# carrenD/Medical-Cross-Modality-Domain-Adaptation

Measured on AMD Instinct MI355X. Metric: training slices/sec (256x256x3, B=16/GPU) joint segmenter+GAN step (1 dis update on B MR + B CT, clip, 1 gen update on B CT), higher is better.
Workload: dtype f32; 1 GPU; BASELINE configs[3]: train_gan.py --phase train-gan joint step, B=16/GPU per domain, f32, dropout .75, mask critic on; global_batch=16, per_gpu_batch=16, parallelism=dp1, step_capture=False

## Files before the change

include/pnp_hip.h:

```cpp
#ifndef PNP_HIP_H
#define PNP_HIP_H

#include <stddef.h>
#include <stdint.h>

#ifdef __cplusplus
extern "C" {
#endif

#define PNP_OK 0
#define PNP_EINVAL (-1)
#define PNP_ELAUNCH (-2)
#define PNP_EWORKSPACE (-3)
#define PNP_ECOMM (-4)

#define PNP_DTYPE_F32 0
#define PNP_DTYPE_BF16 1
#define PNP_DTYPE_F64 2

#define PNP_PAD_ZERO 0
#define PNP_PAD_SYMMETRIC 1

int pnp_abi_version(void);
const char* pnp_last_error(void);
// ... 30 lines not shown

int32_t pnp_conv2d_fwd_stats_parts(const pnp_conv_geom* g);
int pnp_conv2d_fwd_stats(const float* x, const float* w, float* y, const pnp_conv_geom* g,
                         float keep_prob, uint64_t seed, uint32_t stream_id,
                         const float* shift , float* parts, size_t parts_bytes, void* stream);
int32_t pnp_conv2d_fwd_stats_ws_parts(const pnp_conv_geom* g);
int pnp_conv2d_fwd_stats_ws(const float* x, const float* w, float* y, const pnp_conv_geom* g,
                            float keep_prob, uint64_t seed, uint32_t stream_id,
                            const float* shift , float* parts, size_t parts_bytes,
                            void* workspace, size_t workspace_bytes, void* stream);
int32_t pnp_conv2d_wino_chosen(const pnp_conv_geom* g, int32_t kind);
int32_t pnp_conv2d_wino_mode(int32_t mode);
int32_t pnp_conv2d_wino_tile(int32_t tile);
int32_t pnp_conv2d_wino_x3(int32_t mode);
int32_t pnp_conv2d_x3_direct(int32_t mode);
size_t pnp_conv2d_wino_filter_bytes(int32_t C, int32_t K);
int pnp_conv2d_wino_filter_bind(const float* w, int32_t kind, float* U, size_t bytes);
void pnp_weights_changed(const void* lo, const void* hi);
void pnp_conv2d_wino_filter_stats(int64_t* hits, int64_t* fills, int32_t reset);
int32_t pnp_conv2d_wino_wgrad_mode(int32_t mode);

int pnp_bn_fold(const float* gamma, const float* beta, const float* mean, const float* var, float* scale, float* shift,
                int32_t C, float eps, void* stream);
int pnp_conv2d_fwd_bn(const float* x, const float* w, float* y, const pnp_conv_geom* g,
                      float keep_prob, uint64_t seed, uint32_t stream_id,
                      const float* scale, const float* shift, const float* shortcut , int32_t Cs, float alpha,
                      void* stream);
int pnp_conv2d_fwd_bn_ws(const float* x, const float* w, float* y, const pnp_conv_geom* g,
                         float keep_prob, uint64_t seed, uint32_t stream_id,
                         const float* scale, const float* shift, const float* shortcut , int32_t Cs, float alpha,
// ... 160 lines not shown
```

medical-cross-modality-domain-adaptation_amd/_lib.py:

```python
import ctypes
import os

import torch

from ctypes import POINTER, c_char_p, c_float, c_int, c_int32, c_int64, c_size_t, c_uint32, c_uint64, c_void_p

_HERE = os.path.dirname(os.path.abspath(__file__))
LIB_PATH = os.environ.get("PNP_LIB") or os.path.join(_HERE, "libpnp_hip.so")

PAD_ZERO = 0
PAD_SYMMETRIC = 1
OPT_CHUNK = 1024
DTYPE_F32, DTYPE_BF16, DTYPE_F64 = 0, 1, 2
COMM_ID_BYTES = 128
ABI_VERSION = 4


class ConvGeom(ctypes.Structure):
    _fields_ = [(n, c_int32) for n in
                ("N", "H", "W", "C", "K", "R", "S", "OH", "OW", "stride", "dil", "pad_t", "pad_l", "pad_mode", "dtype")]

    def key(self):
        return tuple(getattr(self, f) for f, _ in self._fields_)

# ... 30 lines not shown
    "pnp_conv2d_fwd_ws": (c_int, [_F, _F, _F, _G, c_float, c_uint64, c_uint32, c_void_p, c_size_t, c_void_p]),
    "pnp_conv2d_fwd_stats_parts": (c_int32, [_G]),
    "pnp_conv2d_fwd_stats": (c_int, [_F, _F, _F, _G, c_float, c_uint64, c_uint32, _F, _F, c_size_t, c_void_p]),
    "pnp_bn_stats_finish": (c_int, [_F, c_int32, _F, _F, _F, _F, _F, c_int64, c_int32, c_float, c_void_p]),
    "pnp_bn_fold": (c_int, [_F, _F, _F, _F, _F, _F, c_int32, c_float, c_void_p]),
    "pnp_conv2d_fwd_bn": (c_int, [_F, _F, _F, _G, c_float, c_uint64, c_uint32, _F, _F, _F, c_int32, c_float, c_void_p]),
    "pnp_conv2d_fwd_bn_ws": (c_int, [_F, _F, _F, _G, c_float, c_uint64, c_uint32, _F, _F, _F, c_int32, c_float, c_void_p, c_size_t, c_void_p]),
    "pnp_conv2d_fwd_stats_ws_parts": (c_int32, [_G]),
    "pnp_conv2d_fwd_stats_ws": (c_int, [_F, _F, _F, _G, c_float, c_uint64, c_uint32, _F, _F, c_size_t, c_void_p, c_size_t, c_void_p]),
    "pnp_conv2d_wino_chosen": (c_int32, [_G, c_int32]),
    "pnp_conv2d_wino_mode": (c_int32, [c_int32]),
    "pnp_conv2d_wino_wgrad_mode": (c_int32, [c_int32]),
    "pnp_conv2d_wino_tile": (c_int32, [c_int32]),
    "pnp_conv2d_wino_x3": (c_int32, [c_int32]),
    "pnp_conv2d_x3_direct": (c_int32, [c_int32]),
    "pnp_conv2d_wino_filter_bytes": (c_size_t, [c_int32, c_int32]),
    "pnp_conv2d_wino_filter_bind": (c_int, [c_void_p, c_int32, c_void_p, c_size_t]),
    "pnp_weights_changed": (None, [c_void_p, c_void_p]),
    "pnp_conv2d_wino_filter_stats": (None, [POINTER(c_int64), POINTER(c_int64), c_int32]),
    "pnp_conv2d_fwd_naive": (c_int, [_F, _F, _F, _G, c_void_p]),
    "pnp_dropout": (c_int, [_F, _F, c_size_t, c_float, c_uint64, c_uint32, c_void_p]),
    "pnp_bn_workspace_bytes": (c_size_t, [c_int64, c_int32]),
    "pnp_bn_stats": (c_int, [_F, _F, _F, c_int64, c_int32, c_void_p, c_size_t, c_void_p]),
    "pnp_bn_stats_update": (c_int, [_F, _F, _F, _F, _F, c_int64, c_int32, c_float, c_void_p, c_size_t, c_void_p]),
    "pnp_bn_update_moving": (c_int, [_F, _F, _F, _F, c_int64, c_int32, c_float, c_void_p]),
    "pnp_bn_apply": (c_int, [_F, _F, _F, _F, _F, _F, c_int32, _F, c_int64, c_int32, c_float, c_float, c_void_p]),
    "pnp_bn_bwd": (c_int, [_F, _F, _F, _F, _F, _F, _F, _F, _F, _F, _F, c_int32, c_int64, c_int32, c_float, c_float, c_int32,
                           c_float, c_uint64, c_uint32, c_void_p, c_size_t, c_void_p]),
    "pnp_bn_bwd_acc": (c_int, [_F, _F, _F, _F, _F, _F, _F, _F, _F, _F, _F, _F, _F, c_int32, c_int64, c_int32, c_float, c_float, c_int32,
                               c_float, c_uint64, c_uint32, c_void_p, c_size_t, c_void_p]),
# ... 112 lines not shown
```

medical-cross-modality-domain-adaptation_amd/csrc/conv_common.h:

```cpp
#pragma once
#include "pnp_common.h"

namespace pnpconv {

constexpr int BK = 32;
constexpr int NTHREADS = 256;
#ifndef PNP_CONV_ABLATE
#define PNP_CONV_ABLATE 0
#endif
constexpr int kAblate = PNP_CONV_ABLATE;

struct ConvArgs {
    const float* x;
    const float* w;
    float* y;
    int N, H, W, C, K, R, S, OH, OW, stride, dil, pad_t, pad_l, pad_mode;
    int ups;
    int M;
    int Kred;
    int OHW;
    int nblk_m, nblk_n;
    int gn;
    int nsplit, chunks_per_split;
    long long split_stride;
// ... 288 lines not shown
    size_t wt_off;
};
int plan_phases(const pnp_conv_geom* g, DgradPhase* ph);
pnp_conv_geom phase_geom(const pnp_conv_geom* g, const DgradPhase& p);
bool n16_geom_ok(const pnp_conv_geom* g);
bool n16_wgrad_ok(const pnp_conv_geom* g);
int launch_n16_fwd(const ConvArgs& a, int kind, hipStream_t st);
int n16_wgrad_blocks(const pnp_conv_geom* g);
int launch_n16_wgrad(const ConvArgs& a, float* part, hipStream_t st);
bool wino_eligible(const pnp_conv_geom* g);
bool x3d_chosen(const pnp_conv_geom* g);
bool x3d_chosen(const ConvArgs& a);
int x3d_stats_parts(const pnp_conv_geom* g);
size_t x3d_filter_bytes(int C, int K);
int launch_x3_direct(const ConvArgs& a, int kind, bool flip_transpose, void* ws, size_t ws_bytes, hipStream_t st);
bool wino_chosen(const pnp_conv_geom* g);
int wino_tile(const pnp_conv_geom* g);
size_t wino_workspace_bytes(const pnp_conv_geom* g);
int wino_stats_parts(const pnp_conv_geom* g);
int launch_wino(const ConvArgs& a, int kind, bool flip_transpose, void* ws, size_t ws_bytes, hipStream_t st);
bool wino_wgrad_chosen(const pnp_conv_geom* g);
int wino_wgrad_tile(const pnp_conv_geom* g);
size_t wino_wgrad_workspace_bytes(const pnp_conv_geom* g);
int launch_wino_wgrad(const ConvArgs& a, float* dw, int accumulate, void* ws, size_t ws_bytes, hipStream_t st);
#ifndef PNP_X3_SW
#define PNP_X3_SW 32
#endif
constexpr int X3_SW = PNP_X3_SW;
static_assert(X3_SW == 16 || X3_SW == 32, "stage width");
bool wino_x3_dims_ok(int T, int C, int K);
// ... 10 lines not shown
```

medical-cross-modality-domain-adaptation_amd/csrc/conv_igemm.hip:

```cpp
#include "conv_common.h"
#include "conv_mma.h"

using namespace pnpconv;

#ifdef PNP_TRACE
constexpr int TRACE_WG = 512, TRACE_N = 192;
__device__ unsigned long long g_trace[TRACE_WG][TRACE_N];
#define PNP_TRACE_MARK(slot)                                                                             \
    do {                                                                                                 \
        const unsigned tr_ = blockIdx.x - (gridDim.x > 4352u ? 4096u : 0u);        \
        if (threadIdx.x == 0 && tr_ < (unsigned)TRACE_WG && (slot) < TRACE_N) g_trace[tr_][(slot)] = __builtin_readcyclecounter(); \
    } while (0)
extern "C" int pnp_debug_trace_read(void* host, size_t bytes) {
    if (bytes > sizeof(unsigned long long) * TRACE_WG * TRACE_N) bytes = sizeof(unsigned long long) * TRACE_WG * TRACE_N;
    return hipMemcpyFromSymbol(host, HIP_SYMBOL(g_trace), bytes, 0, hipMemcpyDeviceToHost) == hipSuccess ? 0 : -1;
}
#else
#define PNP_TRACE_MARK(slot) do { } while (0)
#endif

namespace {

template <int BN, bool VEC>
struct BLoader {
// ... 1895 lines not shown
        flops += 2.0 * rows * g->C * (double)(p.T * p.U * g->K);
        bytes += 4.0 * (rows * g->C + (double)p.T * p.U * g->K * g->C);
    }
    ga.nph = n;
    if (n == 0) return PNP_OK;
    bytes += 4.0 * (double)g->N * g->OH * g->OW * g->K;
    PnpProfScope ps(PNP_PROF_CONV_DGRAD, st, flops, bytes, "conv_dgrad_phases_kernel<128, %d, %d, %d>", bn, narrow ? 4 : 2, narrow ? 1 : 2);
    if (narrow) hipLaunchKernelGGL((conv_dgrad_phases_kernel<128, 32, 4, 1>), dim3((unsigned)blk), dim3(NTHREADS), 0, st, ga);
    else hipLaunchKernelGGL((conv_dgrad_phases_kernel<128, 64, 2, 2>), dim3((unsigned)blk), dim3(NTHREADS), 0, st, ga);
    PNP_CHECK_LAUNCH("conv_dgrad_phases_kernel");
    return PNP_OK;
}

}

extern "C" {

static int fwd_split(const pnp_conv_geom* g) {
    if (g->pad_mode != PNP_PAD_ZERO) return 1;
    const long long M = (long long)g->N * g->OH * g->OW;
    const int tile = choose_tile(M, g->K);
    const int bn = tile == 0 ? 128 : (tile == 1 ? 64 : 32);
    if ((long long)pnp_cdiv(M, 128) * pnp_cdiv(g->K, bn) > 128) return 1;
    return choose_split(M, g->K, g->R * g->S * g->C, tile);
}

size_t pnp_conv2d_fwd_workspace_bytes(const pnp_conv_geom* g) {
    if (!g) return 0;
    if (wino_chosen(g)) return wino_workspace_bytes(g);
    const int ns = fwd_split(g);
    const size_t split = ns > 1 ? (size_t)ns * g->N * g->OH * g->OW * g->K * sizeof(float) : 0;
    const size_t x3d = x3d_chosen(g) ? x3d_filter_bytes(g->C, g->K) : 0;
    return split > x3d ? split : x3d;
}

int pnp_conv2d_fwd(const float* x, const float* w, float* y, const pnp_conv_geom* g, float keep_prob, uint64_t seed,
                   uint32_t stream_id, void* stream) {
    return pnp_conv2d_fwd_ws(x, w, y, g, keep_prob, seed, stream_id, nullptr, 0, stream);
}

int pnp_conv2d_fwd_ws(const float* x, const float* w, float* y, const pnp_conv_geom* g, float keep_prob, uint64_t seed,
                      uint32_t stream_id, void* workspace, size_t workspace_bytes, void* stream) {
    if (int e = check_geom(g, "pnp_conv2d_fwd")) return e;
    PNP_REQUIRE(x && w && y, "pnp_conv2d_fwd: null pointer");
    PNP_REQUIRE(keep_prob > 0.f, "pnp_conv2d_fwd: keep_prob must be > 0");
    ConvArgs a = make_args(x, w, y, g);
    if (keep_prob < 1.f) {
        a.do_drop = 1;
        a.drop_keep = keep_prob;
        a.drop_key = pnp_drop_key(seed, stream_id);
        a.drop_thresh = pnp_drop_thresh(keep_prob);
        a.sp = pnp_step_params_ptr(); a.drop_sid = stream_id;
    }
    if (n16_geom_ok(g)) return launch_n16_fwd(a, 0, (hipStream_t)stream);
    if (narrow_fwd_ok(g, nullptr)) return launch_narrow(x, w, y, g, a, (hipStream_t)stream);
    if (wino_chosen(g)) {
        if (workspace && workspace_bytes >= wino_workspace_bytes(g)) return launch_wino(a, 0, false, workspace, workspace_bytes, (hipStream_t)stream);
        return launch_fwd<0>(a, (hipStream_t)stream, nullptr);
    }
    if (x3d_chosen(a) && workspace && workspace_bytes >= x3d_filter_bytes(a.C, a.K))
        return launch_x3_direct(a, 0, false, workspace, workspace_bytes, (hipStream_t)stream);
    float* split_ws = (workspace && workspace_bytes >= pnp_conv2d_fwd_workspace_bytes(g) && pnp_conv2d_fwd_workspace_bytes(g) > 0)
                          ? (float*)workspace : nullptr;
    return launch_fwd<0>(a, (hipStream_t)stream, split_ws);
}

static int fwd_stats_impl(const float* x, const float* w, float* y, const pnp_conv_geom* g, float keep_prob, uint64_t seed,
                          uint32_t stream_id, const float* shift, float* parts, size_t parts_bytes, void* workspace, size_t workspace_bytes,
                          void* stream, bool with_ws);

int32_t pnp_conv2d_fwd_stats_parts(const pnp_conv_geom* g) {
    if (!g || check_geom(g, "pnp_conv2d_fwd_stats_parts") != PNP_OK) return 0;
    if (n16_geom_ok(g) || narrow_fwd_ok(g, nullptr) || fwd_split(g) > 1) return 0;
    const long long M = (long long)g->N * g->OH * g->OW;
    const int tile = choose_tile(M, g->K);
    return pnp_cdiv(M, 128) * ((tile == 0 || tile == 1) ? 2 : 4);
}

int pnp_conv2d_fwd_stats(const float* x, const float* w, float* y, const pnp_conv_geom* g, float keep_prob, uint64_t seed,
                         uint32_t stream_id, const float* shift, float* parts, size_t parts_bytes, void* stream) {
    return fwd_stats_impl(x, w, y, g, keep_prob, seed, stream_id, shift, parts, parts_bytes, nullptr, 0, stream, false);
}

int32_t pnp_conv2d_fwd_stats_ws_parts(const pnp_conv_geom* g) {
    if (!g || check_geom(g, "pnp_conv2d_fwd_stats_ws_parts") != PNP_OK) return 0;
    if (wino_chosen(g)) return wino_stats_parts(g);
    if (x3d_chosen(g) && !n16_geom_ok(g) && !narrow_fwd_ok(g, nullptr)) return x3d_stats_parts(g);
    return pnp_conv2d_fwd_stats_parts(g);
}

int pnp_conv2d_fwd_stats_ws(const float* x, const float* w, float* y, const pnp_conv_geom* g, float keep_prob, uint64_t seed,
                            uint32_t stream_id, const float* shift, float* parts, size_t parts_bytes, void* workspace,
                            size_t workspace_bytes, void* stream) {
    return fwd_stats_impl(x, w, y, g, keep_prob, seed, stream_id, shift, parts, parts_bytes, workspace, workspace_bytes, stream, true);
}

static int fwd_stats_impl(const float* x, const float* w, float* y, const pnp_conv_geom* g, float keep_prob, uint64_t seed,
                          uint32_t stream_id, const float* shift, float* parts, size_t parts_bytes, void* workspace, size_t workspace_bytes,
                          void* stream, bool with_ws) {
    if (int e = check_geom(g, "pnp_conv2d_fwd_stats")) return e;
    PNP_REQUIRE(x && w && y && parts, "pnp_conv2d_fwd_stats: null pointer");
    PNP_REQUIRE(keep_prob > 0.f, "pnp_conv2d_fwd_stats: keep_prob must be > 0");
    const bool wino = with_ws && wino_chosen(g);
    if (wino) PNP_REQUIRE(workspace && workspace_bytes >= wino_workspace_bytes(g), "pnp_conv2d_fwd_stats_ws: workspace too small (pnp_conv2d_fwd_workspace_bytes)");
    const bool x3d = with_ws && !wino && x3d_chosen(g) && !n16_geom_ok(g) && !narrow_fwd_ok(g, nullptr);
    if (x3d) PNP_REQUIRE(workspace && workspace_bytes >= x3d_filter_bytes(g->C, g->K), "pnp_conv2d_fwd_stats_ws: workspace too small (pnp_conv2d_fwd_workspace_bytes)");
    const int nparts = wino ? wino_stats_parts(g) : (x3d ? x3d_stats_parts(g) : pnp_conv2d_fwd_stats_parts(g));
    PNP_REQUIRE(nparts > 0, "pnp_conv2d_fwd_stats: no epilogue statistics for this geometry (pnp_conv2d_fwd_stats_parts == 0)");
    if (parts_bytes < (size_t)nparts * 2 * g->K * sizeof(float)) {
        pnp_set_error("pnp_conv2d_fwd_stats: parts buffer too small (%zu < %zu)", parts_bytes, (size_t)nparts * 2 * g->K * sizeof(float));
        return PNP_EWORKSPACE;
    }
    ConvArgs a = make_args(x, w, y, g);
    if (keep_prob < 1.f) {
        a.do_drop = 1;
        a.drop_keep = keep_prob;
        a.drop_key = pnp_drop_key(seed, stream_id);
        a.drop_thresh = pnp_drop_thresh(keep_prob);
        a.sp = pnp_step_params_ptr(); a.drop_sid = stream_id;
    }
    a.stat_ws = parts;
    a.stat_shift = shift;
    if (wino) return launch_wino(a, 0, false, workspace, workspace_bytes, (hipStream_t)stream);
    if (x3d) return launch_x3_direct(a, 0, false, workspace, workspace_bytes, (hipStream_t)stream);
    return launch_fwd<0>(a, (hipStream_t)stream);
}

int pnp_bn_fold(const float* gamma, const float* beta, const float* mean, const float* var, float* scale, float* shift, int32_t C,
                float eps, void* stream) {
    PNP_REQUIRE(gamma && beta && mean && var && scale && shift && C > 0, "pnp_bn_fold: bad argument");
    hipLaunchKernelGGL(bn_fold_kernel, dim3((unsigned)pnp_cdiv(C, 256)), dim3(256), 0, (hipStream_t)stream, gamma, beta, mean, var, scale,
                       shift, C, eps);
    PNP_CHECK_LAUNCH("bn_fold_kernel");
    return PNP_OK;
}

int pnp_conv2d_fwd_bn(const float* x, const float* w, float* y, const pnp_conv_geom* g, float keep_prob, uint64_t seed,
                      uint32_t stream_id, const float* scale, const float* shift, const float* shortcut, int32_t Cs, float alpha,
                      void* stream) {
// ... 58 lines not shown

static bool dgrad_x3d(const pnp_conv_geom* g, pnp_conv_geom* d) {
    if (g->stride != 1 || g->pad_mode != PNP_PAD_ZERO) return false;
    *d = dgrad_as_conv(g);
    return d->pad_t >= 0 && d->pad_l >= 0 && !wino_chosen(d) && !n16_geom_ok(d) && !narrow_fwd_ok(d, nullptr) && x3d_chosen(d);
}

static size_t dgrad_ws_base(const pnp_conv_geom* g);

size_t pnp_conv2d_dgrad_workspace_bytes(const pnp_conv_geom* g) {
    if (!g) return 0;
    const size_t b = dgrad_ws_base(g);
    pnp_conv_geom d;
    if (dgrad_x3d(g, &d)) {
        const size_t f = x3d_filter_bytes(d.C, d.K);
        return b > f ? b : f;
    }
    return b;
}

static size_t dgrad_ws_base(const pnp_conv_geom* g) {
    {
        pnp_conv_geom d;
        if (dgrad_wino(g, &d)) return wino_workspace_bytes(&d);
    }
    size_t b = (size_t)g->R * g->S * g->C * g->K * sizeof(float);
    b = (b + 255) & ~(size_t)255;
    size_t outb = (size_t)g->N * g->H * g->W * g->C * sizeof(float);
    if (g->pad_mode == PNP_PAD_SYMMETRIC) {
        outb = (size_t)g->N * (g->H + 2 * g->pad_t) * (g->W + 2 * g->pad_l) * g->C * sizeof(float);
// ... 41 lines not shown
    float* wt = (float*)workspace;
    size_t woff = ((size_t)g->R * g->S * g->C * g->K * sizeof(float) + 255) & ~(size_t)255;
    const size_t dx_elems = (size_t)g->N * g->H * g->W * g->C;
    auto add_residual = [&](float* out, const float* res) -> int {
        return res ? pnp_axpby(res, out, dx_elems, 1.f, 1.f, stream) : PNP_OK;
    };
    DgradPhase ph[16];
    const int nph = plan_phases(g, ph);
    if (nph > 0) {
        const bool symp = g->pad_mode == PNP_PAD_SYMMETRIC;
        const int Ho = symp ? g->H + 2 * g->pad_t : g->H, Wo = symp ? g->W + 2 * g->pad_l : g->W;
        float* outp = symp ? (float*)((char*)workspace + woff) : dx;
        size_t poff = woff;
        if (symp) poff += ((size_t)g->N * Ho * Wo * g->C * sizeof(float) + 255) & ~(size_t)255;
        float* split_ws = (workspace_bytes > poff) ? (float*)((char*)workspace + poff) : nullptr;
        dim3 tgp((unsigned)pnp_cdiv(g->K, 32), (unsigned)pnp_cdiv(g->C, 32), (unsigned)(g->R * g->S));
        hipLaunchKernelGGL(flip_transpose_phase_kernel, tgp, dim3(256), 0, st, w, wt, g->R, g->S, g->C, g->K, g->stride);
        PNP_CHECK_LAUNCH("flip_transpose_phase_kernel");
        if (phases_in_one_launch(g, ph, nph)) {
            if (int e = launch_phase_group(dy, wt, outp, g, ph, nph, Ho, Wo, st)) return e;
        } else {
            for (int i = 0; i < nph; ++i) {
                const DgradPhase& p = ph[i];
                if (p.I == 0 || p.J == 0) continue;
                const pnp_conv_geom d = phase_geom(g, p);
                ConvArgs a = make_args(dy, wt + p.wt_off, outp, &d);
                a.o_s = g->stride; a.o_H = Ho; a.o_W = Wo; a.o_h0 = p.h0; a.o_w0 = p.w0;
                if (int e = launch_fwd<1>(a, st, split_ws)) return e;
            }
        }
// ... 215 lines not shown
```

medical-cross-modality-domain-adaptation_amd/csrc/conv_x3_direct.hip:

```cpp
#include <atomic>
#include <cstdlib>
#include "conv_common.h"

using namespace pnpconv;

namespace {

typedef __bf16 bf16x8 __attribute__((ext_vector_type(8)));
typedef __bf16 bf16x4 __attribute__((ext_vector_type(4)));
typedef __attribute__((address_space(3))) void lds_void;

constexpr int TH = 16, TW = 16, PH = TH + 2, PW = TW + 2, NPX = PH * PW;
constexpr int ROWB = 64;
constexpr int PLANE_P = NPX * ROWB;
constexpr int PATCH = 3 * PLANE_P;
constexpr int NF = 3;
constexpr int LDS_BYTES = 2 * PATCH + NF * 3 * 64 * ROWB;
constexpr int NPL = 192;
constexpr int NPI = (NPX * 8 + NPL - 1) / NPL;

__device__ __forceinline__ int swz(int row) { return (row >> 2) & 3; }
__device__ __forceinline__ void wait_lgkm0() { asm volatile("s_waitcnt lgkmcnt(0)" ::: "memory"); }
__device__ __forceinline__ void wait_vm0() { asm volatile("s_waitcnt vmcnt(0)" ::: "memory"); }
template <int N>
// ... 287 lines not shown
    const int tap = r % 9; r /= 9;
    const int hf = r % NH, kb = r / NH;
    const int ic = hf * 32 + i, oc = kb * KW + o;
    const float v = FLIP ? w[((size_t)(8 - tap) * K + oc) * C + ic] : w[((size_t)tap * C + ic) * K + oc];
    const __bf16 b0 = (__bf16)v;
    const float r1 = v - (float)b0;
    const __bf16 b1 = (__bf16)r1;
    const float r2 = r1 - (float)b1;
    const __bf16 b2 = (__bf16)r2;
    const size_t base = ((((size_t)kb * NH + hf) * 9 + tap) * 3) * ((size_t)KW * 32) + (size_t)o * 32 + i;
    w3[base] = __builtin_bit_cast(unsigned short, b0);
    w3[base + (size_t)KW * 32] = __builtin_bit_cast(unsigned short, b1);
    w3[base + 2 * (size_t)KW * 32] = __builtin_bit_cast(unsigned short, b2);
}

std::atomic<int> g_x3d_mode{-1};

int x3d_mode() {
    int m = g_x3d_mode.load(std::memory_order_relaxed);
    if (m < 0) {
        m = getenv("PNP_X3_DIRECT") ? atoi(getenv("PNP_X3_DIRECT")) : 1;
        g_x3d_mode.store(m, std::memory_order_relaxed);
    }
    return m;
}

bool dims_ok(int R, int S, int stride, int dil, int C, int K, int OH, int OW, long long M) {
    if (!(R == 3 && S == 3 && stride == 1 && dil == 1 && (C == 32 || C == 64) && (K == 32 || K == 64 || K == 128) && (OH % TH) == 0 && (OW % TW) == 0 &&
          M * (long long)K < (1ll << 30)))
        return false;
    return x3d_mode() >= 2 || (M / (TH * TW)) * (K == 32 ? 1 : K / 64) >= 256;
}

}

namespace pnpconv {

bool x3d_chosen(const pnp_conv_geom* g) {
    return x3d_mode() > 0 && g->dtype == PNP_DTYPE_F32 && (g->pad_mode == PNP_PAD_ZERO || (g->pad_t == 0 && g->pad_l == 0)) && dims_ok(g->R, g->S, g->stride, g->dil, g->C, g->K, g->OH, g->OW, (long long)g->N * g->OH * g->OW);
}

bool x3d_chosen(const ConvArgs& a) {
    return x3d_mode() > 0 && a.dtype == PNP_DTYPE_F32 && (a.pad_mode == PNP_PAD_ZERO || (a.pad_t == 0 && a.pad_l == 0)) && a.ups == 1 && a.o_s == 0 && a.y_h == nullptr && a.ep_scale == nullptr &&
           dims_ok(a.R, a.S, a.stride, a.dil, a.C, a.K, a.OH, a.OW, a.M);
}

int x3d_stats_parts(const pnp_conv_geom* g) { return (int)(((long long)g->N * g->OH * g->OW) / 64); }

size_t x3d_filter_bytes(int C, int K) { return (size_t)9 * C * K * 6; }

int launch_x3_direct(const ConvArgs& a, int kind, bool flip_transpose, void* ws, size_t ws_bytes, hipStream_t st) {
// ... 30 lines not shown
        if (KW == 32) { if (kind == 0) X3D_LAUNCH(2, 32, 0); else X3D_LAUNCH(2, 32, 1); }
        else { if (kind == 0) X3D_LAUNCH(2, 64, 0); else X3D_LAUNCH(2, 64, 1); }
    }
#undef X3D_LAUNCH
    PNP_CHECK_LAUNCH("conv_x3_direct_kernel");
    return PNP_OK;
}

}

extern "C" int32_t pnp_conv2d_x3_direct(int32_t mode) {
    const int prev = x3d_mode();
    if (mode >= 0) g_x3d_mode.store(mode > 2 ? 2 : mode, std::memory_order_relaxed);
    return prev;
}
```

medical-cross-modality-domain-adaptation_amd/kernels.py:

```python
import ctypes
import os
import weakref

import torch

from . import _lib
from ._lib import ConvGeom, PAD_SYMMETRIC, PAD_ZERO, check

_ws_cache = {}


_raw_stream = getattr(torch._C, "_cuda_getCurrentRawStream", None)
_raw_device = getattr(torch._C, "_cuda_getDevice", None)


def _stream_ptr():
    if _raw_stream is not None and _raw_device is not None:
        return _raw_stream(_raw_device())
    return torch.cuda.current_stream().cuda_stream


def _stream():
    return ctypes.c_void_p(_stream_ptr())

# ... 96 lines not shown
    return int(_lib.load().pnp_conv2d_wino_wgrad_mode(int(mode)))


def wino_tile(tile=-1):
    return int(_lib.load().pnp_conv2d_wino_tile(int(tile)))


def wino_x3(mode=-1):
    return int(_lib.load().pnp_conv2d_wino_x3(int(mode)))


def x3_direct(mode=-1):
    return int(_lib.load().pnp_conv2d_x3_direct(int(mode)))


def wino_chosen(g, kind=0):
    return int(_lib.load().pnp_conv2d_wino_chosen(ctypes.byref(g), int(kind)))


U_CACHE = os.environ.get("PNP_WINOGRAD_UCACHE", "1") != "0"
_u_cache = {}


def _u_drop(key, ref=None):
    ent = _u_cache.get(key)
    if ent is None or (ref is not None and ent[0] is not ref):
        return
    del _u_cache[key]
    if ent[1] is not None:
        try:
# ... 702 lines not shown
```

Before: 276.1 slices/s.

## Add strided 3-split bf16 direct conv kernel for forward and phase-decomposed dgrad

Adds a new strided-convolution route that decomposes stride-s convolutions into s*s phases and runs them on the existing warp-specialised bf16x3 split-precision direct conv pipeline, for both forward and transposed (dgrad) layers. A filter-packing kernel reorders weights per phase into the 3-way bf16 split layout, and routing, workspace sizing and stats-part queries are extended to pick it by default when shape constraints and an occupancy heuristic hold. This aims to replace slower generic implicit-GEMM paths for strided discriminator/encoder convolutions with matrix-core work, at the cost of a per-call filter repack and added routing complexity.

Result: faster. 281.0 slices/s (median of 6 runs) (+1.8%).

```diff
diff --git a/include/pnp_hip.h b/include/pnp_hip.h
--- a/include/pnp_hip.h
+++ b/include/pnp_hip.h
@@ -68,6 +68,7 @@
 int32_t pnp_conv2d_wino_tile(int32_t tile);
 int32_t pnp_conv2d_wino_x3(int32_t mode);
 int32_t pnp_conv2d_x3_direct(int32_t mode);
+int32_t pnp_conv2d_x3_strided(int32_t mode);
 size_t pnp_conv2d_wino_filter_bytes(int32_t C, int32_t K);
 int pnp_conv2d_wino_filter_bind(const float* w, int32_t kind, float* U, size_t bytes);
 void pnp_weights_changed(const void* lo, const void* hi);
diff --git a/medical-cross-modality-domain-adaptation_amd/_lib.py b/medical-cross-modality-domain-adaptation_amd/_lib.py
--- a/medical-cross-modality-domain-adaptation_amd/_lib.py
+++ b/medical-cross-modality-domain-adaptation_amd/_lib.py
@@ -68,6 +68,7 @@
     "pnp_conv2d_wino_tile": (c_int32, [c_int32]),
     "pnp_conv2d_wino_x3": (c_int32, [c_int32]),
     "pnp_conv2d_x3_direct": (c_int32, [c_int32]),
+    "pnp_conv2d_x3_strided": (c_int32, [c_int32]),
     "pnp_conv2d_wino_filter_bytes": (c_size_t, [c_int32, c_int32]),
     "pnp_conv2d_wino_filter_bind": (c_int, [c_void_p, c_int32, c_void_p, c_size_t]),
     "pnp_weights_changed": (None, [c_void_p, c_void_p]),
diff --git a/medical-cross-modality-domain-adaptation_amd/csrc/conv_common.h b/medical-cross-modality-domain-adaptation_amd/csrc/conv_common.h
--- a/medical-cross-modality-domain-adaptation_amd/csrc/conv_common.h
+++ b/medical-cross-modality-domain-adaptation_amd/csrc/conv_common.h
@@ -326,6 +326,9 @@
 int x3d_stats_parts(const pnp_conv_geom* g);
 size_t x3d_filter_bytes(int C, int K);
 int launch_x3_direct(const ConvArgs& a, int kind, bool flip_transpose, void* ws, size_t ws_bytes, hipStream_t st);
+bool x3s_chosen(const pnp_conv_geom* g, int kind);
+size_t x3s_filter_bytes(const pnp_conv_geom* g);
+int launch_x3_strided(const ConvArgs& a, const pnp_conv_geom* g, int kind, void* ws, size_t ws_bytes, hipStream_t st);
 bool wino_chosen(const pnp_conv_geom* g);
 int wino_tile(const pnp_conv_geom* g);
 size_t wino_workspace_bytes(const pnp_conv_geom* g);
diff --git a/medical-cross-modality-domain-adaptation_amd/csrc/conv_igemm.hip b/medical-cross-modality-domain-adaptation_amd/csrc/conv_igemm.hip
--- a/medical-cross-modality-domain-adaptation_amd/csrc/conv_igemm.hip
+++ b/medical-cross-modality-domain-adaptation_amd/csrc/conv_igemm.hip
@@ -1933,6 +1933,15 @@
 
 }
 
+static int fwd_x3_route(const pnp_conv_geom* g) {
+    if (wino_chosen(g) || n16_geom_ok(g) || narrow_fwd_ok(g, nullptr)) return 0;
+    if (x3d_chosen(g)) return 1;
+    return x3s_chosen(g, 0) ? 2 : 0;
+}
+static size_t fwd_x3_bytes(const pnp_conv_geom* g, int route) {
+    return route == 1 ? x3d_filter_bytes(g->C, g->K) : (route == 2 ? x3s_filter_bytes(g) : 0);
+}
+
 extern "C" {
 
 static int fwd_split(const pnp_conv_geom* g) {
@@ -1949,7 +1958,7 @@
     if (wino_chosen(g)) return wino_workspace_bytes(g);
     const int ns = fwd_split(g);
     const size_t split = ns > 1 ? (size_t)ns * g->N * g->OH * g->OW * g->K * sizeof(float) : 0;
-    const size_t x3d = x3d_chosen(g) ? x3d_filter_bytes(g->C, g->K) : 0;
+    const size_t x3d = fwd_x3_bytes(g, fwd_x3_route(g));
     return split > x3d ? split : x3d;
 }
 
@@ -1977,8 +1986,11 @@
         if (workspace && workspace_bytes >= wino_workspace_bytes(g)) return launch_wino(a, 0, false, workspace, workspace_bytes, (hipStream_t)stream);
         return launch_fwd<0>(a, (hipStream_t)stream, nullptr);
     }
-    if (x3d_chosen(a) && workspace && workspace_bytes >= x3d_filter_bytes(a.C, a.K))
-        return launch_x3_direct(a, 0, false, workspace, workspace_bytes, (hipStream_t)stream);
+    if (const int x3 = fwd_x3_route(g)) {
+        if (workspace && workspace_bytes >= fwd_x3_bytes(g, x3))
+            return x3 == 1 ? launch_x3_direct(a, 0, false, workspace, workspace_bytes, (hipStream_t)stream)
+                           : launch_x3_strided(a, g, 0, workspace, workspace_bytes, (hipStream_t)stream);
+    }
     float* split_ws = (workspace && workspace_bytes >= pnp_conv2d_fwd_workspace_bytes(g) && pnp_conv2d_fwd_workspace_bytes(g) > 0)
                           ? (float*)workspace : nullptr;
     return launch_fwd<0>(a, (hipStream_t)stream, split_ws);
@@ -2004,7 +2016,7 @@
 int32_t pnp_conv2d_fwd_stats_ws_parts(const pnp_conv_geom* g) {
     if (!g || check_geom(g, "pnp_conv2d_fwd_stats_ws_parts") != PNP_OK) return 0;
     if (wino_chosen(g)) return wino_stats_parts(g);
-    if (x3d_chosen(g) && !n16_geom_ok(g) && !narrow_fwd_ok(g, nullptr)) return x3d_stats_parts(g);
+    if (fwd_x3_route(g)) return x3d_stats_parts(g);
     return pnp_conv2d_fwd_stats_parts(g);
 }
 
@@ -2022,8 +2034,9 @@
     PNP_REQUIRE(keep_prob > 0.f, "pnp_conv2d_fwd_stats: keep_prob must be > 0");
     const bool wino = with_ws && wino_chosen(g);
     if (wino) PNP_REQUIRE(workspace && workspace_bytes >= wino_workspace_bytes(g), "pnp_conv2d_fwd_stats_ws: workspace too small (pnp_conv2d_fwd_workspace_bytes)");
-    const bool x3d = with_ws && !wino && x3d_chosen(g) && !n16_geom_ok(g) && !narrow_fwd_ok(g, nullptr);
-    if (x3d) PNP_REQUIRE(workspace && workspace_bytes >= x3d_filter_bytes(g->C, g->K), "pnp_conv2d_fwd_stats_ws: workspace too small (pnp_conv2d_fwd_workspace_bytes)");
+    const int x3 = (with_ws && !wino) ? fwd_x3_route(g) : 0;
+    const bool x3d = x3 != 0;
+    if (x3d) PNP_REQUIRE(workspace && workspace_bytes >= fwd_x3_bytes(g, x3), "pnp_conv2d_fwd_stats_ws: workspace too small (pnp_conv2d_fwd_workspace_bytes)");
     const int nparts = wino ? wino_stats_parts(g) : (x3d ? x3d_stats_parts(g) : pnp_conv2d_fwd_stats_parts(g));
     PNP_REQUIRE(nparts > 0, "pnp_conv2d_fwd_stats: no epilogue statistics for this geometry (pnp_conv2d_fwd_stats_parts == 0)");
     if (parts_bytes < (size_t)nparts * 2 * g->K * sizeof(float)) {
@@ -2041,7 +2054,8 @@
     a.stat_ws = parts;
     a.stat_shift = shift;
     if (wino) return launch_wino(a, 0, false, workspace, workspace_bytes, (hipStream_t)stream);
-    if (x3d) return launch_x3_direct(a, 0, false, workspace, workspace_bytes, (hipStream_t)stream);
+    if (x3d) return x3 == 1 ? launch_x3_direct(a, 0, false, workspace, workspace_bytes, (hipStream_t)stream)
+                            : launch_x3_strided(a, g, 0, workspace, workspace_bytes, (hipStream_t)stream);
     return launch_fwd<0>(a, (hipStream_t)stream);
 }
 
@@ -2130,6 +2144,10 @@
     pnp_conv_geom d;
     if (dgrad_x3d(g, &d)) {
         const size_t f = x3d_filter_bytes(d.C, d.K);
+        return b > f ? b : f;
+    }
+    if (x3s_chosen(g, 1)) {
+        const size_t f = x3s_filter_bytes(g);
         return b > f ? b : f;
     }
     return b;
@@ -2201,6 +2219,11 @@
         size_t poff = woff;
         if (symp) poff += ((size_t)g->N * Ho * Wo * g->C * sizeof(float) + 255) & ~(size_t)255;
         float* split_ws = (workspace_bytes > poff) ? (float*)((char*)workspace + poff) : nullptr;
+        if (x3s_chosen(g, 1)) {
+            ConvArgs a = make_args(dy, w, dx, g);
+            if (int e = launch_x3_strided(a, g, 1, workspace, workspace_bytes, st)) return e;
+            return add_residual(dx, residual);
+        }
         dim3 tgp((unsigned)pnp_cdiv(g->K, 32), (unsigned)pnp_cdiv(g->C, 32), (unsigned)(g->R * g->S));
         hipLaunchKernelGGL(flip_transpose_phase_kernel, tgp, dim3(256), 0, st, w, wt, g->R, g->S, g->C, g->K, g->stride);
         PNP_CHECK_LAUNCH("flip_transpose_phase_kernel");
diff --git a/medical-cross-modality-domain-adaptation_amd/csrc/conv_x3_direct.hip b/medical-cross-modality-domain-adaptation_amd/csrc/conv_x3_direct.hip
--- a/medical-cross-modality-domain-adaptation_amd/csrc/conv_x3_direct.hip
+++ b/medical-cross-modality-domain-adaptation_amd/csrc/conv_x3_direct.hip
@@ -325,6 +325,362 @@
     w3[base + 2 * (size_t)KW * 32] = __builtin_bit_cast(unsigned short, b2);
 }
 
+constexpr int X3S_MAXPH = 16;
+
+struct X3sPhase {
+    int T, U;
+    int ih0, iw0;
+};
+struct X3sGroup {
+    int first_item, tiles_x, tiles_y;
+    int ph0, nph, nst;
+    int o_h0, o_w0;
+    int fbase;
+};
+struct X3sArgs {
+    const float* x;
+    const unsigned short* w3;
+    float* y;
+    int N, H, W, C, K, NH, si;
+    int OHt, OWt, o_s;
+    int ngroups, nitems;
+    unsigned w3_bytes;
+    X3sGroup grp[X3S_MAXPH];
+    X3sPhase ph[X3S_MAXPH];
+    int do_drop;
+    uint32_t drop_thresh, drop_key;
+    float drop_keep;
+    const pnp_step_params* sp;
+    uint32_t drop_sid;
+    float* stat_ws;
+    const float* stat_shift;
+};
+
+__device__ __forceinline__ int x3s_group(const X3sArgs& a, int id) {
+    int gi = 0;
+    for (int i = 1; i < a.ngroups; ++i)
+        if (id >= a.grp[i].first_item) gi = i;
+    return gi;
+}
+
+template <int KIND>
+__global__ void __launch_bounds__(512, 1) conv_x3_direct_kernel_strided(X3sArgs a) {
+    constexpr int KW = 64, TN = 2;
+    constexpr int PLANE_F = KW * ROWB, FSTG = 3 * PLANE_F, NPC = FSTG / 1024;
+    __shared__ __attribute__((aligned(256))) unsigned char lds[LDS_BYTES];
+    unsigned char* const patch0 = lds;
+    unsigned char* const filt0 = lds + 2 * PATCH;
+    const int t = threadIdx.x, lane = t & 63;
+    const int wave = __builtin_amdgcn_readfirstlane(t >> 6);
+    const int KB = a.K / KW, NH = a.NH;
+    int myitems = 0, gstages = 0, nslots = 0;
+    for (int i = blockIdx.x; i < a.nitems; i += gridDim.x) {
+        const X3sGroup& G = a.grp[x3s_group(a, i)];
+        ++myitems;
+        gstages += NH * G.nst;
+        nslots += NH * G.nph;
+    }
+    if (myitems == 0) return;
+    auto item_origin = [&](int it, int& gi, int& kb, int& tile, int& n, int& oh0, int& ow0) {
+        const int id = blockIdx.x + it * gridDim.x;
+        gi = x3s_group(a, id);
+        const X3sGroup& G = a.grp[gi];
+        const int loc = id - G.first_item;
+        tile = loc / KB;
+        kb = loc - tile * KB;
+        n = tile / (G.tiles_x * G.tiles_y);
+        const int r = tile - n * G.tiles_x * G.tiles_y;
+        oh0 = (r / G.tiles_x) * TH;
+        ow0 = (r % G.tiles_x) * TW;
+    };
+    struct Cur { int it, hh, k; };
+
+    if (wave == 4) {
+        const __amdgpu_buffer_rsrc_t rw = make_rsrc(reinterpret_cast<const float*>(a.w3), a.w3_bytes);
+        const int lrow = lane >> 2, lchk = lane & 3;
+        constexpr int PPP = KW / 16;
+        unsigned vo[NPC];
+#pragma unroll
+        for (int i = 0; i < NPC; ++i) {
+            const int row = (i % PPP) * 16 + lrow;
+            vo[i] = (unsigned)((i / PPP) * PLANE_F + row * ROWB + ((lchk ^ swz(row)) << 4));
+        }
+        Cur c{0, 0, 0};
+        int gi, kb, tile, n, oh0, ow0;
+        item_origin(0, gi, kb, tile, n, oh0, ow0);
+        auto issue = [&](int g) {
+            const X3sGroup& G = a.grp[gi];
+            const int stg = G.fbase + (kb * NH + c.hh) * G.nst + c.k;
+            unsigned char* bp = filt0 + (g % NF) * FSTG;
+#pragma unroll
+            for (int i = 0; i < NPC; ++i) dma16(rw, (lds_void*)(bp + i * 1024), vo[i], stg * FSTG);
+            if (++c.k == G.nst) {
+                c.k = 0;
+                if (++c.hh == NH) {
+                    c.hh = 0;
+                    if (++c.it < myitems) item_origin(c.it, gi, kb, tile, n, oh0, ow0);
+                }
+            }
+        };
+#pragma unroll
+        for (int b = 0; b < NF - 1; ++b)
+            if (b < gstages) issue(b);
+        for (int g = 0; g < gstages; ++g) {
+            if (g + NF - 2 < gstages) wait_vm<NPC * (NF - 2)>();
+            else wait_vm0();
+            __builtin_amdgcn_s_barrier();
+            if (g + NF - 1 < gstages) issue(g + NF - 1);
+        }
+        wait_vm0();
+        return;
+    }
+    if (wave > 4) {
+        const int pl = (wave - 5) * 64 + lane;
+        f32x4 st[NPI];
+        Cur lc{0, 0, 0};
+        auto load = [&]() {
+            int gi, kb, tile, n, oh0, ow0;
+            item_origin(lc.it, gi, kb, tile, n, oh0, ow0);
+            const X3sPhase P = a.ph[a.grp[gi].ph0 + lc.k];
+            const int rmax = TH - 1 + P.T, cmax = TW - 1 + P.U;
+#pragma unroll
+            for (int i = 0; i < NPI; ++i) {
+                const int e = pl + i * NPL;
+                const int q = e >> 3, j = e & 7;
+                const int pr = q / PW, pc = q - pr * PW;
+                const int ih = a.si * (oh0 + pr) + P.ih0, iw = a.si * (ow0 + pc) + P.iw0;
+                const bool ok = (e < NPX * 8) & (pr < rmax) & (pc < cmax) & ((unsigned)ih < (unsigned)a.H) & ((unsigned)iw < (unsigned)a.W);
+                f32x4 v = {0.f, 0.f, 0.f, 0.f};
+                if (ok) v = *reinterpret_cast<const f32x4*>(a.x + (((size_t)n * a.H + ih) * a.W + iw) * a.C + lc.hh * 32 + j * 4);
+                st[i] = v;
+            }
+        };
+        auto advance = [&](Cur& c) {
+            const int id = blockIdx.x + c.it * gridDim.x;
+            if (++c.k == a.grp[x3s_group(a, id)].nph) {
+                c.k = 0;
+                if (++c.hh == NH) { c.hh = 0; ++c.it; }
+            }
+        };
+        auto store = [&](int slot) {
+            unsigned char* pb = patch0 + (slot & 1) * PATCH;
+#pragma unroll
+            for (int i = 0; i < NPI; ++i) {
+                const int e = pl + i * NPL;
+                if (e >= NPX * 8) continue;
+                const int q = e >> 3, j = e & 7;
+                bf16x4 hi, mi, lo;
+#pragma unroll
+                for (int c = 0; c < 4; ++c) {
+                    const float v = st[i][c];
+                    const __bf16 h = (__bf16)v;
+                    const float r1 = v - (float)h;
+                    const __bf16 m = (__bf16)r1;
+                    const float r2 = r1 - (float)m;
+                    hi[c] = h; mi[c] = m; lo[c] = (__bf16)r2;
+                }
+                const int off = q * ROWB + (((j >> 1) ^ swz(q)) << 4) + (j & 1) * 8;
+                *reinterpret_cast<bf16x4*>(pb + off) = hi;
+                *reinterpret_cast<bf16x4*>(pb + PLANE_P + off) = mi;
+                *reinterpret_cast<bf16x4*>(pb + 2 * PLANE_P + off) = lo;
+            }
+        };
+        auto taps_of = [&](const Cur& c) {
+            const int id = blockIdx.x + c.it * gridDim.x;
+            const X3sPhase& P = a.ph[a.grp[x3s_group(a, id)].ph0 + c.k];
+            return P.T * P.U;
+        };
+        load();
+        wait_vm0();
+        store(0);
+        advance(lc);
+        if (nslots > 1) load();
+        Cur sc{0, 0, 0};
+        int k = 0, j = 0, ns = taps_of(sc);
+        for (int g = 0; g < gstages; ++g) {
+            if (j == 0) wait_lgkm0();
+            __builtin_amdgcn_s_barrier();
+            if (j == ns - 1) {
+                if (k + 1 < nslots) {
+                    wait_vm0();
+                    store(k + 1);
+                    advance(lc);
+                    if (k + 2 < nslots) load();
+                }
+                ++k;
+                j = 0;
+                advance(sc);
+                if (k < nslots) ns = taps_of(sc);
+            } else {
+                ++j;
+            }
+        }
+        return;
+    }
+    const int l31 = lane & 31, h = lane >> 5;
+    const int prow = l31 >> 4, pcol = (l31 < 16) ? l31 : ((l31 - 16 + 14) & 15);
+    int aq[2];
+#pragma unroll
+    for (int tm = 0; tm < 2; ++tm) aq[tm] = (4 * wave + 2 * tm + prow) * PW + pcol;
+    int woff[TN][2];
+#pragma unroll
+    for (int tn = 0; tn < TN; ++tn)
+#pragma unroll
+        for (int ks = 0; ks < 2; ++ks) woff[tn][ks] = (tn * 32 + l31) * ROWB + (((2 * ks + h) ^ swz(tn * 32 + l31)) << 4);
+    constexpr int kTermX[6] = {2, 1, 0, 1, 0, 0}, kTermW[6] = {0, 1, 2, 0, 1, 0};
+    f32x16 acc[2][TN];
+    bf16x8 xf[2][3][2];
+    bf16x8 xn[3][2];
+    auto x_frag = [&](const unsigned char* A, int dq, int ks, int p, int tm) {
+        const int q = aq[tm] + dq;
+        return *reinterpret_cast<const bf16x8*>(A + p * PLANE_P + q * ROWB + (((2 * ks + h) ^ swz(q)) << 4));
+    };
+    const uint32_t dkey = a.do_drop ? pnp_eff_drop_key(a.drop_key, a.sp, a.drop_sid) : 0u;
+    int g = 0, slot = 0;
+    for (int it = 0; it < myitems; ++it) {
+        int gi, kb, tile, n, oh0, ow0;
+        item_origin(it, gi, kb, tile, n, oh0, ow0);
+        const X3sGroup& G = a.grp[gi];
+#pragma unroll
+        for (int tm = 0; tm < 2; ++tm)
+#pragma unroll
+            for (int tn = 0; tn < TN; ++tn)
+#pragma unroll
+                for (int e = 0; e < 16; ++e) acc[tm][tn][e] = 0.f;
+        for (int hh = 0; hh < NH; ++hh) {
+            for (int pk = 0; pk < G.nph; ++pk, ++slot) {
+                const X3sPhase P = a.ph[G.ph0 + pk];
+                const unsigned char* A = patch0 + (slot & 1) * PATCH;
+                for (int tap = 0, ntap = P.T * P.U; tap < ntap; ++tap, ++g) {
+                    const int tr = tap / P.U, tc = tap - tr * P.U;
+                    const int dq = tr * PW + tc;
+                    wait_lgkm0();
+                    __builtin_amdgcn_s_barrier();
+                    asm volatile("" ::: "memory");
+                    if (tap == 0) {
+#pragma unroll
+                        for (int p = 0; p < 3; ++p)
+#pragma unroll
+                            for (int tm = 0; tm < 2; ++tm) xf[0][p][tm] = x_frag(A, 0, 0, p, tm);
+                    } else {
+#pragma unroll
+                        for (int p = 0; p < 3; ++p)
+#pragma unroll
+                            for (int tm = 0; tm < 2; ++tm) xf[0][p][tm] = xn[p][tm];
+                    }
+                    const unsigned char* B = filt0 + (g % NF) * FSTG;
+                    bf16x8 wf[2][3][TN];
+#pragma unroll
+                    for (int p = 0; p < 3; ++p)
+#pragma unroll
+                        for (int tn = 0; tn < TN; ++tn) wf[0][p][tn] = *reinterpret_cast<const bf16x8*>(B + p * PLANE_F + woff[tn][0]);
+#pragma unroll
+                    for (int p = 0; p < 3; ++p) {
+#pragma unroll
+                        for (int tm = 0; tm < 2; ++tm) xf[1][p][tm] = x_frag(A, dq, 1, p, tm);
+#pragma unroll
+                        for (int tn = 0; tn < TN; ++tn) wf[1][p][tn] = *reinterpret_cast<const bf16x8*>(B + p * PLANE_F + woff[tn][1]);
+                    }
+                    if (tap + 1 < ntap) {
+                        const int nr = (tap + 1) / P.U, nc = tap + 1 - nr * P.U;
+#pragma unroll
+                        for (int p = 0; p < 3; ++p)
+#pragma unroll
+                            for (int tm = 0; tm < 2; ++tm) xn[p][tm] = x_frag(A, nr * PW + nc, 0, p, tm);
+                    }
+#pragma unroll
+                    for (int ks = 0; ks < 2; ++ks)
+#pragma unroll
+                        for (int trm = 0; trm < 6; ++trm)
+#pragma unroll
+                            for (int tm = 0; tm < 2; ++tm)
+#pragma unroll
+                                for (int tn = 0; tn < TN; ++tn)
+                                    acc[tm][tn] = __builtin_amdgcn_mfma_f32_32x32x16_bf16(xf[ks][kTermX[trm]][tm], wf[ks][kTermW[trm]][tn], acc[tm][tn], 0, 0, 0);
+                }
+            }
+        }
+        auto mlin_of = [&](int tm, int i) {
+            const int r = (i & 3) + 8 * (i >> 2) + 4 * h;
+            const int orow = oh0 + 4 * wave + 2 * tm + (r >> 4);
+            const int ocol = ow0 + ((r < 16) ? r : ((r - 16 + 14) & 15));
+            return (n * a.OHt + G.o_h0 + a.o_s * orow) * a.OWt + G.o_w0 + a.o_s * ocol;
+        };
+        int ncol[TN];
+#pragma unroll
+        for (int tn = 0; tn < TN; ++tn) ncol[tn] = kb * KW + tn * 32 + l31;
+#define X3S_FOR                                                      \
+    _Pragma("unroll") for (int tm = 0; tm < 2; ++tm)                 \
+        _Pragma("unroll") for (int tn = 0; tn < TN; ++tn)            \
+            _Pragma("unroll") for (int i = 0; i < 16; ++i)
+        if (a.do_drop) {
+            X3S_FOR {
+                const uint32_t idx = (uint32_t)((size_t)mlin_of(tm, i) * a.K + ncol[tn]);
+                acc[tm][tn][i] = pnp_drop_keep(idx, dkey, a.drop_thresh) ? acc[tm][tn][i] / a.drop_keep : 0.f;
+            }
+        }
+        if (a.stat_ws) {
+            const int part = tile * 4 + wave;
+#pragma unroll
+            for (int tn = 0; tn < TN; ++tn) {
+                const float shift = a.stat_shift ? a.stat_shift[ncol[tn]] : 0.f;
+                float ssum = 0.f, ssq = 0.f;
+#pragma unroll
+                for (int tm = 0; tm < 2; ++tm)
+#pragma unroll
+                    for (int i = 0; i < 16; ++i) {
+                        const float d = acc[tm][tn][i] - shift;
+                        ssum += d;
+                        ssq = fmaf(d, d, ssq);
+                    }
+                const float s_ = ssum + __shfl_xor(ssum, 32, 64);
+                const float q_ = ssq + __shfl_xor(ssq, 32, 64);
+                if (h == 0) {
+                    a.stat_ws[((size_t)part * 2 + 0) * a.K + ncol[tn]] = s_;
+                    a.stat_ws[((size_t)part * 2 + 1) * a.K + ncol[tn]] = q_;
+                }
+            }
+        }
+        const __amdgpu_buffer_rsrc_t ry = make_rsrc(a.y, (unsigned)((size_t)a.N * a.OHt * a.OWt * a.K * 4));
+        X3S_FOR bstore1(ry, (unsigned)(mlin_of(tm, i) * a.K + ncol[tn]) * 4u, acc[tm][tn][i]);
+#undef X3S_FOR
+    }
+}
+
+struct X3sTaps {
+    int ngroups, R, S;
+    int st0[X3S_MAXPH + 1];
+    int tr[64], tc[64];
+};
+template <bool FLIP>
+__global__ void __launch_bounds__(256) x3s_filter_kernel(const float* __restrict__ w, unsigned short* __restrict__ w3, int C, int K, X3sTaps tp) {
+    const int NH = C >> 5, KB = K / 64;
+    const long long total = (long long)KB * NH * tp.st0[tp.ngroups] * 64 * 32;
+    const long long e = (long long)blockIdx.x * 256 + threadIdx.x;
+    if (e >= total) return;
+    const int i = (int)(e & 31), o = (int)((e >> 5) & 63);
+    const int simg = (int)(e >> 11);
+    int gi = 0;
+    for (int q = 1; q < tp.ngroups; ++q)
+        if (simg >= KB * NH * tp.st0[q]) gi = q;
+    const int nst = tp.st0[gi + 1] - tp.st0[gi];
+    const int loc = simg - KB * NH * tp.st0[gi];
+    const int s = loc % nst, khh = loc / nst;
+    const int hf = khh % NH, kb = khh / NH;
+    const int r = tp.tr[tp.st0[gi] + s], c = tp.tc[tp.st0[gi] + s];
+    const int ic = hf * 32 + i, oc = kb * 64 + o;
+    const float v = FLIP ? w[(((size_t)r * tp.S + c) * K + oc) * C + ic] : w[(((size_t)r * tp.S + c) * C + ic) * K + oc];
+    const __bf16 b0 = (__bf16)v;
+    const float r1 = v - (float)b0;
+    const __bf16 b1 = (__bf16)r1;
+    const float r2 = r1 - (float)b1;
+    const __bf16 b2 = (__bf16)r2;
+    const size_t base = (size_t)simg * 3 * 64 * 32 + (size_t)o * 32 + i;
+    w3[base] = __builtin_bit_cast(unsigned short, b0);
+    w3[base + 64 * 32] = __builtin_bit_cast(unsigned short, b1);
+    w3[base + 2 * 64 * 32] = __builtin_bit_cast(unsigned short, b2);
+}
+
 std::atomic<int> g_x3d_mode{-1};
 
 int x3d_mode() {
@@ -343,9 +699,135 @@
     return x3d_mode() >= 2 || (M / (TH * TW)) * (K == 32 ? 1 : K / 64) >= 256;
 }
 
+std::atomic<int> g_x3s_mode{-1};
+
+int x3s_mode() {
+    int m = g_x3s_mode.load(std::memory_order_relaxed);
+    if (m < 0) {
+        m = getenv("PNP_X3_STRIDED") ? atoi(getenv("PNP_X3_STRIDED")) : 1;
+        g_x3s_mode.store(m, std::memory_order_relaxed);
+    }
+    return m;
+}
+
+struct X3sPlan {
+    int ngroups, nitems, stride;
+    X3sGroup grp[X3S_MAXPH];
+    X3sPhase ph[X3S_MAXPH];
+    X3sTaps taps;
+};
+
+bool x3s_plan(const pnp_conv_geom* g, int kind, X3sPlan* pl) {
+    if (x3d_mode() <= 0 || x3s_mode() <= 0 || g->dtype != PNP_DTYPE_F32 || g->pad_mode != PNP_PAD_ZERO || g->dil != 1) return false;
+    const int s = g->stride;
+    if (s < 2 || s > 4 || g->R < s || g->S < s || g->R > 3 * s || g->S > 3 * s) return false;
+    const int Cin = kind == 0 ? g->C : g->K, Kout = kind == 0 ? g->K : g->C;
+    if ((Cin % 32) != 0 || (Kout % 64) != 0) return false;
+    const long long out_elems = kind == 0 ? (long long)g->N * g->OH * g->OW * g->K : (long long)g->N * g->H * g->W * g->C;
+    if (out_elems >= (1ll << 30) || (long long)g->R * g->S > 64) return false;
+    X3sPlan p{};
+    p.stride = s;
+    int ns = 0, items = 0;
+    auto add_group = [&](int GH, int GW, int o_h0, int o_w0) -> bool {
+        if (GH <= 0 || GW <= 0 || (GH % TH) != 0 || (GW % TW) != 0) return false;
+        X3sGroup& G = p.grp[p.ngroups++];
+        G.first_item = items;
+        G.tiles_x = GW / TW; G.tiles_y = GH / TH;
+        G.o_h0 = o_h0; G.o_w0 = o_w0;
+        G.fbase = (Kout / 64) * (Cin / 32) * ns;
+        items += g->N * G.tiles_x * G.tiles_y * (Kout / 64);
+        return true;
+    };
+    if (kind == 0) {
+        if (!add_group(g->OH, g->OW, 0, 0)) return false;
+        X3sGroup& G = p.grp[0];
+        G.ph0 = 0; G.nph = s * s; G.nst = g->R * g->S;
+        p.taps.st0[0] = 0;
+        for (int ra = 0; ra < s; ++ra)
+            for (int cb = 0; cb < s; ++cb) {
+                X3sPhase& P = p.ph[ra * s + cb];
+                P.T = (g->R - ra + s - 1) / s; P.U = (g->S - cb + s - 1) / s;
+                P.ih0 = ra - g->pad_t; P.iw0 = cb - g->pad_l;
+                for (int t = 0; t < P.T; ++t)
+                    for (int u = 0; u < P.U; ++u) { p.taps.tr[ns] = ra + s * t; p.taps.tc[ns] = cb + s * u; ++ns; }
+            }
+        p.taps.st0[1] = ns;
+    } else {
+        DgradPhase dp[16];
+        const int nph = plan_phases(g, dp);
+        if (nph != s * s) return false;
+        for (int i = 0; i < nph; ++i) {
+            const DgradPhase& q = dp[i];
+            if (q.T > 3 || q.U > 3) return false;
+            p.taps.st0[i] = ns;
+            if (!add_group(q.I, q.J, q.h0, q.w0)) return false;
+            X3sGroup& G = p.grp[i];
+            G.ph0 = i; G.nph = 1; G.nst = q.T * q.U;
+            X3sPhase& P = p.ph[i];
+            P.T = q.T; P.U = q.U; P.ih0 = -q.pad_t; P.iw0 = -q.pad_l;
+            for (int t = 0; t < q.T; ++t)
+                for (int u = 0; u < q.U; ++u) { p.taps.tr[ns] = q.pa + s * (q.T - 1 - t); p.taps.tc[ns] = q.pb + s * (q.U - 1 - u); ++ns; }
+        }
+        p.taps.st0[nph] = ns;
+    }
+    if (ns != g->R * g->S) return false;
+    p.nitems = items;
+    p.taps.ngroups = p.ngroups; p.taps.R = g->R; p.taps.S = g->S;
+    if (x3d_mode() < 2 && (items < 256 || !(g->R * g->S >= 4 * s * s || (kind == 1 && Cin <= 64)))) return false;
+    if (pl) *pl = p;
+    return true;
+}
+
 }
 
 namespace pnpconv {
+
+bool x3s_chosen(const pnp_conv_geom* g, int kind) { return x3s_plan(g, kind, nullptr); }
+
+size_t x3s_filter_bytes(const pnp_conv_geom* g) { return (size_t)g->R * g->S * g->C * g->K * 6; }
+
+int launch_x3_strided(const ConvArgs& a, const pnp_conv_geom* g, int kind, void* ws, size_t ws_bytes, hipStream_t st) {
+    X3sPlan pl;
+    if (!x3s_plan(g, kind, &pl)) {
+        pnp_set_error("launch_x3_strided: layer not on this route");
+        return PNP_EINVAL;
+    }
+    const size_t fbytes = x3s_filter_bytes(g);
+    if (!ws || ws_bytes < fbytes) {
+        pnp_set_error("launch_x3_strided: workspace too small (%zu < %zu)", ws_bytes, fbytes);
+        return PNP_EWORKSPACE;
+    }
+    unsigned short* w3 = (unsigned short*)ws;
+    const int cls = prof_class(kind);
+    const int Cin = kind == 0 ? g->C : g->K, Kout = kind == 0 ? g->K : g->C;
+    {
+        const long long total = (long long)g->R * g->S * g->C * g->K;
+        PnpProfScope ps(cls, st, 0.0, 4.0 * total + 6.0 * total, "x3s_filter_kernel<%s>", kind ? "true" : "false");
+        const unsigned blocks = (unsigned)pnp_cdiv(total, 256);
+        if (kind) hipLaunchKernelGGL((x3s_filter_kernel<true>), dim3(blocks), dim3(256), 0, st, a.w, w3, Cin, Kout, pl.taps);
+        else hipLaunchKernelGGL((x3s_filter_kernel<false>), dim3(blocks), dim3(256), 0, st, a.w, w3, Cin, Kout, pl.taps);
+        PNP_CHECK_LAUNCH("x3s_filter_kernel");
+    }
+    X3sArgs x{};
+    x.x = a.x; x.w3 = w3; x.y = a.y;
+    x.N = g->N; x.C = Cin; x.K = Kout; x.NH = Cin / 32;
+    if (kind == 0) { x.H = g->H; x.W = g->W; x.si = g->stride; x.OHt = g->OH; x.OWt = g->OW; x.o_s = 1; }
+    else { x.H = g->OH; x.W = g->OW; x.si = 1; x.OHt = g->H; x.OWt = g->W; x.o_s = g->stride; }
+    x.ngroups = pl.ngroups; x.nitems = pl.nitems;
+    x.w3_bytes = (unsigned)fbytes;
+    for (int i = 0; i < pl.ngroups; ++i) x.grp[i] = pl.grp[i];
+    for (int i = 0; i < X3S_MAXPH; ++i) x.ph[i] = pl.ph[i];
+    x.do_drop = a.do_drop; x.drop_thresh = a.drop_thresh; x.drop_key = a.drop_key; x.drop_keep = a.drop_keep; x.sp = a.sp; x.drop_sid = a.drop_sid;
+    x.stat_ws = kind == 0 ? a.stat_ws : nullptr; x.stat_shift = a.stat_shift;
+    const dim3 grid((unsigned)(pl.nitems > 256 ? 256 : pl.nitems));
+    const double fl = 6.0 * 2.0 * (double)g->N * g->OH * g->OW * g->R * g->S * g->C * g->K;
+    const double by = 4.0 * ((double)g->N * x.H * x.W * Cin + (double)g->N * x.OHt * x.OWt * Kout) + 6.0 * g->R * g->S * g->C * g->K;
+    PnpProfScope ps(cls, st, fl, by, "conv_x3_direct_kernel_strided<%d>", kind);
+    if (kind) hipLaunchKernelGGL((conv_x3_direct_kernel_strided<1>), grid, dim3(512), 0, st, x);
+    else hipLaunchKernelGGL((conv_x3_direct_kernel_strided<0>), grid, dim3(512), 0, st, x);
+    PNP_CHECK_LAUNCH("conv_x3_direct_kernel_strided");
+    return PNP_OK;
+}
 
 bool x3d_chosen(const pnp_conv_geom* g) {
     return x3d_mode() > 0 && g->dtype == PNP_DTYPE_F32 && (g->pad_mode == PNP_PAD_ZERO || (g->pad_t == 0 && g->pad_l == 0)) && dims_ok(g->R, g->S, g->stride, g->dil, g->C, g->K, g->OH, g->OW, (long long)g->N * g->OH * g->OW);
@@ -406,3 +888,9 @@
     if (mode >= 0) g_x3d_mode.store(mode > 2 ? 2 : mode, std::memory_order_relaxed);
     return prev;
 }
+
+extern "C" int32_t pnp_conv2d_x3_strided(int32_t mode) {
+    const int prev = x3s_mode();
+    if (mode >= 0) g_x3s_mode.store(mode > 0 ? 1 : 0, std::memory_order_relaxed);
+    return prev;
+}
diff --git a/medical-cross-modality-domain-adaptation_amd/kernels.py b/medical-cross-modality-domain-adaptation_amd/kernels.py
--- a/medical-cross-modality-domain-adaptation_amd/kernels.py
+++ b/medical-cross-modality-domain-adaptation_amd/kernels.py
@@ -134,6 +134,10 @@
     return int(_lib.load().pnp_conv2d_x3_direct(int(mode)))
 
 
+def x3_strided(mode=-1):
+    return int(_lib.load().pnp_conv2d_x3_strided(int(mode)))
+
+
 def wino_chosen(g, kind=0):
     return int(_lib.load().pnp_conv2d_wino_chosen(ctypes.byref(g), int(kind)))
 
```
